# OpenRendererBenchmark/libYafaRay

Measured on AMD Instinct MI355X. Metric: Mrays/sec (primary+secondary) on the path-tracing hot path, higher is better.
Workload: dtype f32; 1 GPU; 1M-tri diffuse Cornell-box soup 512x512 64spp primary+1-bounce (BASELINE.json metric config); triangles=1000000, width=512, height=512, spp=64, bounces=1, lights=1, parallelism=pixel-tile shard x1, film_reduce=none, kd_nodes=2803313, kd_leaf_refs=3155999, kd_max_depth=27

## Files before the change

libyafaray_amd/csrc/yafgpu_device.hip:

```cpp
#include <hip/hip_runtime.h>

#include <algorithm>
#include <chrono>
#include <cmath>
#include <cstdio>
#include <cstdlib>
#include <cstring>
#include <string>
#include <vector>
#include <map>
#include <mutex>

#include "../../include/yafgpu.h"
#include "kdtree_build.h"
#include "yafgpu_math.h"
#include "yafgpu_shading.h"
#include "yafgpu_texture.h"

namespace yafgpu {

constexpr int kWave = 64;
constexpr int kBlock = 256;
constexpr int kWavesPerBlock = kBlock / kWave;
#ifndef YAFGPU_STACK
// ... 46 lines not shown
                                173, 179, 181, 191, 193, 197, 199, 211, 223, 227};

YG_DEV double scr_halton(const DevScene &sc, int dim, uint32_t n)
{
	double value = 0.0;
	const int *sigma = sc.faure + sc.faure_off[dim];
	const uint32_t base = (uint32_t)c_prims[dim];
	double f, factor, dn = (double)n;
	f = factor = sc.inv_prims[dim];
	while(n > 0)
	{
		value += (double)(sigma[n % base]) * factor;
		dn *= f;
		n = (uint32_t)dn;
		factor *= f;
	}
	return fmax(1.0e-36, fmin(1.0, value));
}

YG_DEV bool bound_cross(const DevScene &sc, V3 from, V3 dir, V3 inv_dir, float dist, float &enter, float &leave)
{
	const V3 a0 = mk(sc.blo[0], sc.blo[1], sc.blo[2]), a1 = mk(sc.bhi[0], sc.bhi[1], sc.bhi[2]);
	const V3 p = from - a0;
	float lmin = -1e38f, lmax = 1e38f, ltmin, ltmax;
	if(dir.x != 0.f)
	{
		const float inv = inv_dir.x;
		if(inv > 0.f) { lmin = -p.x * inv; lmax = ((a1.x - a0.x) - p.x) * inv; }
		else { lmin = ((a1.x - a0.x) - p.x) * inv; lmax = -p.x * inv; }
		if((lmax < 0.f) || (lmin > dist)) return false;
	}
	if(dir.y != 0.f)
	{
		const float inv = inv_dir.y;
		if(inv > 0.f) { ltmin = -p.y * inv; ltmax = ((a1.y - a0.y) - p.y) * inv; }
		else { ltmin = ((a1.y - a0.y) - p.y) * inv; ltmax = -p.y * inv; }
		lmin = smax(ltmin, lmin);
		lmax = smin(ltmax, lmax);
		if((lmax < 0.f) || (lmin > dist)) return false;
	}
	if(dir.z != 0.f)
	{
		const float inv = inv_dir.z;
		if(inv > 0.f) { ltmin = -p.z * inv; ltmax = ((a1.z - a0.z) - p.z) * inv; }
		else { ltmin = ((a1.z - a0.z) - p.z) * inv; ltmax = -p.z * inv; }
		lmin = smax(ltmin, lmin);
		lmax = smin(ltmax, lmax);
		if((lmax < 0.f) || (lmin > dist)) return false;
	}
	if((lmin <= lmax) && (lmax >= 0.f) && (lmin <= dist)) { enter = lmin; leave = lmax; return true; }
	return false;
}

YG_DEV bool tri_test(const float4 r0, const float4 r1, const float4 r2, V3 from, V3 dir, float &t, float &u, float &v)
{
	const V3 a = mk(r0.x, r0.y, r0.z), e1 = mk(r1.x, r1.y, r1.z), e2 = mk(r2.x, r2.y, r2.z);
	const float eps = r0.w;
	const V3 pvec = cross(dir, e2);
	const float det = dot(e1, pvec);
	if(det > -eps && det < eps) return false;
	const float inv_det = 1.f / det;
	const V3 tvec = from - a;
	u = dot(tvec, pvec) * inv_det;
	if(u < 0.f || u > 1.f) return false;
	const V3 qvec = cross(tvec, e1);
	v = dot(dir, qvec) * inv_det;
	if((v < 0.f) || ((u + v) > 1.f)) return false;
	t = dot(e2, qvec) * inv_det;
	if(t < eps) return false;
	return true;
}

YG_DEV bool tri_test_flat(const float4 r0, const float4 r1, const float4 r2, V3 from, V3 dir, float &t, float &u, float &v)
{
	const V3 a = mk(r0.x, r0.y, r0.z), e1 = mk(r1.x, r1.y, r1.z), e2 = mk(r2.x, r2.y, r2.z);
	const float eps = r0.w;
	const V3 pvec = cross(dir, e2);
	const float det = dot(e1, pvec);
	const bool det_ok = !(det > -eps && det < eps);
	const float inv_det = 1.f / det;
	const V3 tvec = from - a;
	u = dot(tvec, pvec) * inv_det;
	const bool u_ok = !(u < 0.f || u > 1.f);
	const V3 qvec = cross(tvec, e1);
	v = dot(dir, qvec) * inv_det;
	const bool v_ok = !((v < 0.f) || ((u + v) > 1.f));
	t = dot(e2, qvec) * inv_det;
	return det_ok && u_ok && v_ok && !(t < eps);
}

struct LaneStack
{
	uint2 *col;
	int sp, lo;
	YG_DEV void reset() { sp = 0; lo = 0; }
	YG_DEV bool empty() const { return sp == lo; }
	YG_DEV bool lost() const { return lo > 0; }
	YG_DEV void push(uint32_t node, float tmax)
	{
		col[(sp & (kStack - 1)) * kWave] = make_uint2(node, __float_as_uint(tmax));
		++sp;
		lo = max(lo, sp - kStack);
	}
	YG_DEV void pop(uint32_t &node, float &tmax)
	{
		--sp;
		const uint2 e = col[(sp & (kStack - 1)) * kWave];
		node = e.x; tmax = __uint_as_float(e.y);
	}
};

YG_DEV float restart_from(float tmin, float tmax)
{
	return (tmax > tmin) ? tmax : tmax + fmaxf(fabsf(tmax) * 1.2e-7f, 1e-30f);
}

YG_DEV void get_surface(const DevScene &sc, int ti, V3 hitp, float bu, float bv, SurfPt &sp)
{
	const float4 g = sc.tri_ng[ti];
	sp.ng = mk(g.x, g.y, g.z);
	if(sc.tri_vn != nullptr && __float_as_uint(g.w) != 0u)
	{
		const float u = 1.f - bu - bv, v = bu, w = bv;
		const float4 na = sc.tri_vn[3 * ti], nb = sc.tri_vn[3 * ti + 1], nc = sc.tri_vn[3 * ti + 2];
		sp.n = normalize(mk(na.x, na.y, na.z) * u + mk(nb.x, nb.y, nb.z) * v + mk(nc.x, nc.y, nc.z) * w);
	}
	else sp.n = sp.ng;
	sp.mat = (int)(__float_as_uint(sc.tri[3 * ti + 1].w) & 0x3FFFFFFFu);
	sp.p = hitp;
	create_cs(sp.n, sp.nu, sp.nv);
}

constexpr int kTsMaxDepth = 8;
YG_DEV bool kd_trace_ts(const DevScene &sc, LaneStack &stk, uint32_t *seen , V3 from, V3 dir, float ray_tmin, float dist,
                        int max_depth, Col &filt)
{
	filt = mkc(1.f, 1.f, 1.f);
	float a, b;
	if(sc.n_nodes == 0u) return false;
	const V3 inv_dir = mk(1.f / dir.x, 1.f / dir.y, 1.f / dir.z);
	if(!bound_cross(sc, from, dir, inv_dir, dist, a, b)) return false;
	const float t_exit = b;
	float tmin = smax(a, 0.f), tmax = t_exit;
	uint32_t node = 0u;
	int depth = 0, n_seen = 0;
	stk.reset();
	for(;;)
	{
		if(dist < tmin) break;
		uint2 nd = sc.nodes[node];
		while((nd.y & 3u) != 3u)
		{
			const int axis = (int)(nd.y & 3u);
			const float split = __uint_as_float(nd.x);
			const float o = comp(from, axis), d = comp(dir, axis);
			const float tplane = (split - o) * comp(inv_dir, axis);
			const bool below = (o < split) || (o == split && d <= 0.f);
			const uint32_t left = node + 1u, right = nd.y >> 2;
			const uint32_t near_c = below ? left : right, far_c = below ? right : left;
			if(!(tplane <= tmax) || tplane <= 0.f) node = near_c;
			else if(tplane < tmin) node = far_c;
			else { stk.push(far_c, tmax); node = near_c; tmax = tplane; }
			nd = sc.nodes[node];
		}
		const uint32_t np = nd.y >> 2, first = nd.x;
		for(uint32_t i = 0; i < np; ++i)
		{
			const uint32_t ti = sc.refs[first + i];
			const float4 r0 = sc.tri[3u * ti], r1 = sc.tri[3u * ti + 1u], r2 = sc.tri[3u * ti + 2u];
			float t, u, v;
			if(!tri_test(r0, r1, r2, from, dir, t, u, v)) continue;
			const uint32_t vis = __float_as_uint(r1.w) >> 30;
			if(!(t < dist && t >= ray_tmin && (vis == 0u || vis == 2u))) continue;
			const yafgpu_material &m = sc.mats[__float_as_uint(r1.w) & 0x3FFFFFFFu];
			if(!mat_is_transparent(m)) return true;
			bool known = false;
			for(int k = 0; k < n_seen; ++k) known = known || (seen[k * kWave] == ti);
			if(known) continue;
			if(depth >= max_depth) return true;
			if(n_seen <= kTsMaxDepth) seen[(n_seen++) * kWave] = ti;
			SurfPt sp;
			get_surface(sc, (int)ti, from + dir * t, u, v, sp);
			if(m.n_nodes > 0 && sc.tex.nodes != nullptr)
			{
				TexPoint tp; tex_point(sc.tex, (int)ti, u, v, sp.p, sp.n, sp.ng, tp);
				yafgpu_material tmp; mat_resolve(sc.tex, sc.cam, m, tp, tmp);
				filt = filt * mat_transparency(tmp, sp, dir);
			}
			else filt = filt * mat_transparency(m, sp, dir);
			++depth;
		}
		if(stk.empty())
		{
			if(!stk.lost() || tmax >= t_exit) break;
			tmin = restart_from(tmin, tmax); tmax = t_exit; node = 0u; stk.reset();
			continue;
		}
		tmin = tmax;
		stk.pop(node, tmax);
	}
	return false;
}

enum : int { kStPrimary = 0, kStFirst = 1, kStDepth = 2 };

YG_DEV int round2int(double v) { return (int)(v + (.5 - 1.4e-11)); }

YG_DEV uint32_t wave_sum(uint32_t v)
{
#pragma unroll
	for(int o = 32; o > 0; o >>= 1) v += __shfl_xor(v, o, kWave);
	return v;
}

}
#include "yafgpu_wavefront.h"
#ifndef YAFGPU_VARIANT_TU
namespace yafgpu {

__global__ __launch_bounds__(kBlock) void combine_kernel(const float *planes, float *film, int w, int h)
{
	const size_t n = (size_t)w * (size_t)h;
	const size_t stride = n * YAFGPU_FILM_CHANNELS;
	for(size_t i = (size_t)blockIdx.x * blockDim.x + threadIdx.x; i < n; i += (size_t)gridDim.x * blockDim.x)
	{
		const int x = (int)(i % (size_t)w), y = (int)(i / (size_t)w);
#pragma unroll
// ... 181 lines not shown
		}
		case 17:
		{
			if(n_in < 4) break;
			const uint32_t k = __float_as_uint(x[3]);
			if(k >= (uint32_t)sc.n_lights || sc.lights[k].type != YAFGPU_LIGHT_DIRECTIONAL || n_out < 8) break;
			Col c = mkc(0.f, 0.f, 0.f); V3 d = mk(0.f, 0.f, 0.f); float tmax = 0.f;
			const bool ok = directionallight_illuminate(sc.lights[k], mk(x[0], x[1], x[2]), c, d, tmax);
			o[0] = ok ? 1.f : 0.f;
			o[1] = ok ? d.x : 0.f; o[2] = ok ? d.y : 0.f; o[3] = ok ? d.z : 0.f; o[4] = ok ? tmax : 0.f; o[5] = ok ? c.r : 0.f; o[6] = ok ? c.g : 0.f; o[7] = ok ? c.b : 0.f;
			break;
		}
		case 18:
		{
			if(n_in < 3) break;
			const uint32_t k = __float_as_uint(x[2]);
			if(k >= (uint32_t)sc.n_lights || sc.lights[k].type != YAFGPU_LIGHT_SUN || n_out < 9) break;
			Col c = mkc(0.f, 0.f, 0.f); V3 d = mk(0.f, 0.f, 0.f); float tmax = 0.f, pdf = 0.f;
			const bool ok = sunlight_illum_sample(sc.lights[k], x[0], x[1], d, tmax, pdf, c);
			o[0] = ok ? 1.f : 0.f;
			o[1] = d.x; o[2] = d.y; o[3] = d.z; o[4] = tmax; o[5] = pdf; o[6] = c.r; o[7] = c.g; o[8] = c.b;
			break;
		}
		case 19:
		{
			if(n_in < 4) break;
			const uint32_t k = __float_as_uint(x[3]);
			if(k >= (uint32_t)sc.n_lights || sc.lights[k].type != YAFGPU_LIGHT_SUN || n_out < 6) break;
			Col c = mkc(0.f, 0.f, 0.f); float t = 0.f, ipdf = 0.f;
			const bool ok = sunlight_intersect(sc.lights[k], mk(x[0], x[1], x[2]), t, c, ipdf);
			o[0] = ok ? 1.f : 0.f; o[1] = t; o[2] = ipdf; o[3] = c.r; o[4] = c.g; o[5] = c.b;
			break;
		}
		case 20:
		{
			if(n_in < 6) break;
			const uint32_t k = __float_as_uint(x[5]);
			if(k >= (uint32_t)sc.n_lights || sc.lights[k].type != YAFGPU_LIGHT_SPHERE || n_out < 9) break;
			Col c = mkc(0.f, 0.f, 0.f); V3 d = mk(0.f, 0.f, 0.f); float tmax = 0.f, pdf = 0.f;
			const bool ok = spherelight_illum_sample(sc.lights[k], mk(x[0], x[1], x[2]), x[3], x[4], d, tmax, pdf, c);
			o[0] = ok ? 1.f : 0.f;
			o[1] = ok ? d.x : 0.f; o[2] = ok ? d.y : 0.f; o[3] = ok ? d.z : 0.f; o[4] = ok ? tmax : 0.f; o[5] = ok ? pdf : 0.f;
			o[6] = ok ? c.r : 0.f; o[7] = ok ? c.g : 0.f; o[8] = ok ? c.b : 0.f;
			break;
		}
		case 21:
		{
			if(n_in < 7) break;
			const uint32_t k = __float_as_uint(x[6]);
			if(k >= (uint32_t)sc.n_lights || sc.lights[k].type != YAFGPU_LIGHT_SPHERE || n_out < 3) break;
			float d_1 = 0.f, d_2 = 0.f;
			const bool ok = sphere_intersect(mk(x[0], x[1], x[2]), mk(x[3], x[4], x[5]), vec3(sc.lights[k].position), sc.lights[k].square_radius, d_1, d_2);
			o[0] = ok ? 1.f : 0.f; o[1] = d_1; o[2] = ok ? d_2 : 0.f;
			break;
		}
		default: break;
	}
}

}

using namespace yafgpu;

static float host_fsin(float x);
static thread_local std::string g_err;
static int fail(int code, const std::string &msg) { g_err = msg; return code; }
#define HIP_OK(expr) do { hipError_t e_ = (expr); if(e_ != hipSuccess) return fail(-100, std::string(#expr) + ": " + hipGetErrorString(e_)); } while(0)

template<typename T> struct DevMem
{
	T *p = nullptr; size_t cap = 0;
	DevMem() = default;
	DevMem(const DevMem &) = delete; DevMem &operator=(const DevMem &) = delete;
	~DevMem() { if(p) (void)hipFree(p); }
	hipError_t alloc(size_t count) { return hipMalloc((void **)&p, std::max<size_t>(count, 1) * sizeof(T)); }
	hipError_t reserve(size_t count, hipStream_t stream)
	{
		if(p && count <= cap) return hipSuccess;
		hipError_t e = hipStreamSynchronize(stream);
		if(e != hipSuccess) return e;
		if(p) (void)hipFree(p);
		p = nullptr; cap = 0;
		if((e = alloc(count)) != hipSuccess) { p = nullptr; return e; }
		cap = count;
		return hipSuccess;
	}
	operator T *() const { return p; }
};
struct Stream
{
	hipStream_t s = nullptr;
	Stream() = default;
	Stream(const Stream &) = delete; Stream &operator=(const Stream &) = delete;
	~Stream() { if(s) (void)hipStreamDestroy(s); }
	hipError_t create() { return s ? hipSuccess : hipStreamCreateWithFlags(&s, hipStreamNonBlocking); }
	operator hipStream_t() const { return s; }
};
struct Event
{
	hipEvent_t e = nullptr;
	Event() = default;
	Event(const Event &) = delete; Event &operator=(const Event &) = delete;
	~Event() { if(e) (void)hipEventDestroy(e); }
	hipError_t create(unsigned flags = hipEventDisableTiming) { return e ? hipSuccess : hipEventCreateWithFlags(&e, flags); }
	operator hipEvent_t() const { return e; }
};
// ... 137 lines not shown
	}
	auto *s = new yafgpu_scene();
	{
		std::vector<char> used((size_t)d->n_materials, 0);
		for(int i = 0; i < d->n_tris; ++i) used[(size_t)d->tri_mat[i]] = 1;
		for(int i = 0; i < d->n_materials; ++i)
		{
			if(!used[(size_t)i]) continue;
			const yafgpu_material &m = d->materials[i];
			s->mat_mask |= 1u << (uint32_t)m.type;
			if(m.bsdf_flags & kVolumetric) s->has_volumetric = true;
			if(m.bsdf_flags & (kSpecular | kFilter)) s->has_specular = true;
			if(m.anisotropic) s->has_aniso = true;
			s->max_add_depth = std::max(s->max_add_depth, std::min(std::max(m.additional_depth, 0), 15));
			if(m.bsdf_flags & kGlossy) s->has_glossy = true;
			if(m.type == YAFGPU_MAT_ROUGH_GLASS) s->has_glossy_two = true;
			if((m.type == YAFGPU_MAT_SHINYDIFFUSE && m.is_transparent) || ((m.type == YAFGPU_MAT_GLASS || m.type == YAFGPU_MAT_ROUGH_GLASS) && m.fake_shadow)) s->has_transparent = true;
		}
	}
	const auto t0 = std::chrono::steady_clock::now();
	{
		bool on_device = d->build_on_device > 0 || (d->build_on_device == 0 && d->n_tris >= 65536);
		if(const char *e = std::getenv("YAFGPU_BUILD")) on_device = std::strcmp(e, "device") == 0;
		if(on_device)
		{
			std::string err;
			const int brc = build_kdtree_device_retry(d->verts, d->n_tris, kDepthCap, s->tree, &err);
			if(brc == -2 || brc == -3) build_kdtree(d->verts, d->n_tris, kDepthCap, d->build_threads, s->tree);
			else if(brc) { delete s; return fail(-20, err); }
		}
		else build_kdtree(d->verts, d->n_tris, kDepthCap, d->build_threads, s->tree);
	}
	s->info.build_seconds = s->tree.build_seconds;
	s->info.n_nodes = (uint32_t)s->tree.nodes.size();
	s->info.n_leaf_refs = (uint32_t)s->tree.refs.size();
	s->info.max_depth = (uint32_t)s->tree.max_depth;
	s->info.n_tris = (uint32_t)d->n_tris;
	const auto t1 = std::chrono::steady_clock::now();

	const size_t nt = (size_t)d->n_tris;
	std::vector<float4> rec(3 * nt), ng(nt), vn;
	bool any_smooth = false;
	for(size_t i = 0; i < nt; ++i)
	{
		const float *v = d->verts + 9 * i;
		const float e1[3] = {v[3] - v[0], v[4] - v[1], v[5] - v[2]}, e2[3] = {v[6] - v[0], v[7] - v[1], v[8] - v[2]};
		const float l1 = std::sqrt(e1[0] * e1[0] + e1[1] * e1[1] + e1[2] * e1[2]);
		const float l2 = std::sqrt(e2[0] * e2[0] + e2[1] * e2[1] + e2[2] * e2[2]);
		const float eps = (float)((double)0.1f * 0.00005 * (double)std::max(l1, l2));
		const uint32_t mat = (uint32_t)d->tri_mat[i];
		const uint32_t vis = (uint32_t)d->materials[mat].visibility & 3u;
		float mw; const uint32_t packed = mat | (vis << 30); std::memcpy(&mw, &packed, 4);
		rec[3 * i] = make_float4(v[0], v[1], v[2], eps);
		rec[3 * i + 1] = make_float4(e1[0], e1[1], e1[2], mw);
		rec[3 * i + 2] = make_float4(e2[0], e2[1], e2[2], 0.f);
		float n[3] = {e1[1] * e2[2] - e1[2] * e2[1], e1[2] * e2[0] - e1[0] * e2[2], e1[0] * e2[1] - e1[1] * e2[0]};
		float len = n[0] * n[0] + n[1] * n[1] + n[2] * n[2];
		if(len != 0.f) { len = 1.0f / std::sqrt(len); n[0] *= len; n[1] *= len; n[2] *= len; }
		bool smooth = false;
		if(d->vnormals)
		{
			const float *q = d->vnormals + 9 * i;
			for(int k = 0; k < 9; ++k) if(q[k] != 0.f) smooth = true;
		}
		float sw; const uint32_t sbits = smooth ? 1u : 0u; std::memcpy(&sw, &sbits, 4);
		ng[i] = make_float4(n[0], n[1], n[2], sw);
		any_smooth |= smooth;
	}
	if(any_smooth)
	{
		vn.resize(3 * nt);
		for(size_t i = 0; i < nt; ++i)
		{
			const float *q = d->vnormals + 9 * i;
			for(int c = 0; c < 3; ++c)
			{
				float x = q[3 * c], y = q[3 * c + 1], z = q[3 * c + 2];
				if(x == 0.f && y == 0.f && z == 0.f) { x = ng[i].x; y = ng[i].y; z = ng[i].z; }
				vn[3 * i + (size_t)c] = make_float4(x, y, z, 0.f);
			}
		}
	}
	std::vector<int> faure; std::vector<int> foff(50); std::vector<double> invp(50);
	for(int dim = 0; dim < 50; ++dim)
	{
		foff[(size_t)dim] = (int)faure.size();
		std::vector<int> p;
		if(dim < 3) p = {0, 1, 2};
		else faure_perm(kPrimsHost[dim], p);
		faure.insert(faure.end(), p.begin(), p.end());
		char buf[32];
		std::snprintf(buf, sizeof buf, "%.9f", 1.0 / (double)kPrimsHost[dim]);
		invp[(size_t)dim] = std::strtod(buf, nullptr);
	}
	int rc = 0;
	DevScene &dv = s->dev;
	if((rc = upload(s, (const uint2 *)s->tree.nodes.data(), s->tree.nodes.size(), &dv.nodes))) { yafgpu_scene_destroy(s); return rc; }
	{
		const char *e = std::getenv("YAFGPU_TREELET_INLINE");
		TreeletLayout tl;
		if(build_treelets(s->tree.nodes, !(e && std::atoi(e) == 0), tl)) { yafgpu_scene_destroy(s); return fail(-2, "kd-tree too large for the treelet layout"); }
		dv.tl_root = tl.root;
		if((rc = upload(s, (const uint4 *)tl.words.data(), tl.words.size() / 4, &dv.treelets))) { yafgpu_scene_destroy(s); return rc; }
		if((rc = upload(s, (const uint2 *)tl.leaves.data(), tl.leaves.size() / 2, &dv.tl_leaves))) { yafgpu_scene_destroy(s); return rc; }
	}
	if((rc = upload(s, s->tree.refs.data(), s->tree.refs.size(), &dv.refs))) { yafgpu_scene_destroy(s); return rc; }
	if((rc = upload(s, rec.data(), rec.size(), &dv.tri))) { yafgpu_scene_destroy(s); return rc; }
	if((rc = upload(s, ng.data(), ng.size(), &dv.tri_ng))) { yafgpu_scene_destroy(s); return rc; }
// ... 1274 lines not shown
```

libyafaray_amd/csrc/yafgpu_wavefront.h:

```cpp
#pragma once

namespace yafgpu {

constexpr int kWfRecs = 32;

struct WfArgs
{
	RenderArgs ra;
	float4 *state; uint32_t cap;
	float4 *results;
	uint32_t n_paths, pixel_begin, n_pixels;
	const uint32_t *pix_prefix;
	int frames;
	int frame_recs, has_glossy;
	int pix_listed;
	uint32_t *pix_xy;
	const uint32_t *q_closest_in, *q_shadow_in, *q_resume_in;
	uint32_t *q_closest_out, *q_shadow_out, *q_resume_out;
	uint32_t *verdict;
	float4 *shadow_filt;
	int replay, replay_lights;
	int ev_m;
	float4 *hit_cache; int hit_k;
	uint32_t *ev_flags;
// ... 91 lines not shown
		}
		return true;
	}
	r_tmin = ra.rp.min_raydist_auto ? ra.ray_min_dist * smax(1.f, length(sp.p)) : ra.ray_min_dist;
	float W = 0.f;
	BsdfSample bs; bs.s_1 = s_1; bs.s_2 = s_2; bs.pdf = 0.f; bs.flags = kMisFlags; bs.sampled = kNone;
	const Col surf_col = mat_sample(mat, dat, sp, wo, r_dir, bs, W);
	float light_ipdf;
	Col l_col = mkc(0.f, 0.f, 0.f);
	if(YG_LIGHT_IS(light, YAFGPU_LIGHT_SUN)) { if(!(bs.pdf > 1e-6f && sunlight_intersect(light, r_dir, r_tmax, l_col, light_ipdf))) return false; }
	else if(YG_LIGHT_IS(light, YAFGPU_LIGHT_SPHERE)) return false;
	else if(!(bs.pdf > 1e-6f && arealight_intersect(light, sp.p, r_dir, r_tmax, light_ipdf))) return false;
	if(light_ipdf > 1e-6f)
	{
		const float l_pdf = 1.f / light_ipdf;
		const float l_2 = l_pdf * l_pdf, m_2 = bs.pdf * bs.pdf;
		const float w = m_2 / (l_2 + m_2);
		contrib = ((surf_col * (YG_LIGHT_IS(light, YAFGPU_LIGHT_SUN) ? l_col : col3(light.color))) * w) * W;
	}
	return true;
}

YG_DEV float4 &wf_rec(const WfArgs &a, int k, uint32_t slot)
{
	return *(float4 *)((char *)(a.state + (size_t)k * a.cap) + (slot << 4));
}
#define REC(k) wf_rec(a, (k), slot)
YG_DEV uint32_t wf_event(const WfArgs &a, uint32_t slot, uint32_t z19, int path_i)
{
	const uint32_t call = a.ev_m > 1 ? min(z19 >> 24, (uint32_t)a.ev_m - 1u) : 0u;
	return (slot * (uint32_t)a.ev_m + call) * (uint32_t)max(a.ra.rp.path_samples, 1) + (uint32_t)path_i;
}

YG_DEV const yafgpu_material &wf_mat_hit(const DevScene &sc, const SurfPt &sp, int tri, float bu, float bv, yafgpu_material &tmp)
{
	const yafgpu_material &m = sc.mats[sp.mat];
#if YAFGPU_FEAT_TEXTURE
	if(m.n_nodes > 0 && sc.tex.nodes != nullptr)
	{
		TexPoint tp; tex_point(sc.tex, tri, bu, bv, sp.p, sp.n, sp.ng, tp);
		mat_resolve(sc.tex, sc.cam, m, tp, tmp);
		return tmp;
	}
#endif
	return m;
}
YG_DEV bool wf_bump_hit(const DevScene &sc, SurfPt &sp, int tri, float bu, float bv)
{
#if YAFGPU_FEAT_TEXTURE
	const yafgpu_material &m = sc.mats[sp.mat];
	if(m.n_bump <= 0 || !sc.tex.has_bump) return false;
	TexPoint tp; tex_point(sc.tex, tri, bu, bv, sp.p, sp.n, sp.ng, tp);
	const float4 r1 = sc.tri[3 * tri + 1], r2 = sc.tri[3 * tri + 2];
	tex_point_derivatives(sc.tex, tri, mk(r1.x, r1.y, r1.z), mk(r2.x, r2.y, r2.z), sp.n, sp.nu, sp.nv, tp);
	NodeResult stack[kMaxNodes];
	nodes_eval_derivative(sc.tex, sc.tex.nodes + m.bump_first, min(m.n_bump, kMaxNodes), sc.cam, tp, stack);
	apply_bump(sp.n, sp.nu, sp.nv, stack[m.sh_bump].col.r, stack[m.sh_bump].col.g);
	return true;
#else
	(void)sc; (void)sp; (void)tri; (void)bu; (void)bv;
	return false;
#endif
}
YG_DEV void wf_frame_set(SurfPt &sp, const float4 nu)
{
	if(nu.w != 0.f) { sp.nu = v3(nu); sp.nv = normalize(cross(sp.n, sp.nu)); }
}
YG_DEV void wf_frame_parked(const WfArgs &a, uint32_t slot, int vertex, SurfPt &sp)
{
#if YAFGPU_FEAT_TEXTURE
	if(a.ra.sc.tex.has_bump) wf_frame_set(sp, REC(24 + vertex));
#else
	(void)a; (void)slot; (void)vertex; (void)sp;
#endif
}
YG_DEV const yafgpu_material &wf_mat_parked(const WfArgs &a, uint32_t slot, int vertex, const SurfPt &sp, yafgpu_material &tmp)
{
	const yafgpu_material &m = a.ra.sc.mats[sp.mat];
#if YAFGPU_FEAT_TEXTURE
	if(m.n_nodes > 0 && a.ra.sc.tex.nodes != nullptr)
	{
		const float4 r = REC(22 + vertex);
		return wf_mat_hit(a.ra.sc, sp, (int)ubits(r.x), r.y, r.z, tmp);
	}
#endif
	return m;
}

struct Ctl { Col col; int pc, stage, dl_on_sp0, depth, path_i, level, incl, add, mask2; };
YG_DEV uint32_t pack_ctl(const Ctl &c) { return (uint32_t)c.pc | ((uint32_t)c.stage << 2) | ((uint32_t)c.dl_on_sp0 << 4) | ((uint32_t)c.level << 5) | ((uint32_t)c.depth << 8) | ((uint32_t)c.add << 12) | ((uint32_t)c.incl << 16) | (((uint32_t)c.path_i & 0x1fffu) << 17) | ((uint32_t)c.mask2 << 30); }
YG_DEV Ctl load_ctl(const WfArgs &a, uint32_t slot)
{
	const float4 r = REC(13);
	const uint32_t w = ubits(r.w);
	Ctl c; c.col = c3(r);
	c.pc = (int)(w & 3u); c.stage = (int)((w >> 2) & 3u); c.dl_on_sp0 = (int)((w >> 4) & 1u); c.level = (int)((w >> 5) & 7u);
	c.depth = (int)((w >> 8) & 0xfu); c.add = (int)((w >> 12) & 0xfu); c.incl = (int)((w >> 16) & 1u); c.path_i = (int)((w >> 17) & 0x1fffu); c.mask2 = (int)(w >> 30);
	return c;
}
YG_DEV uint32_t pack_dlc(int li, int l_end, int mask, int is) { return (uint32_t)li | ((uint32_t)l_end << 8) | ((uint32_t)mask << 16) | ((uint32_t)is << 20); }

enum { W_AFTER_CLOSEST, W_AFTER_SHADOW, W_DL_NEXT, W_DL_EVAL, W_DL_DONE, W_RECURSE, W_RETURN, W_EXTEND, W_START_PATH, W_FINISH, W_PARK_CLOSEST, W_PARK_SHADOW,
       W_GLOSSY_NEXT, W_RECURSE_SPEC, W_PARK_BOTH, W_NEXT_VERTEX };

#ifndef YAFGPU_HOT_ACC
#define YAFGPU_HOT_ACC 1
#endif
// ... 1073 lines not shown
		float4 *b = a.state + slot; const size_t c = a.cap;
		b[0 * c] = f4(from, tmin);
		b[1 * c] = f4(dir, tmax);
		b[13 * c] = make_float4(0.f, 0.f, 0.f, fbits((uint32_t)kPcAfterClosest | ((uint32_t)kStPrimary << 2)));
	}
	if(blockIdx.x == 0 && threadIdx.x == 0) { a.cnt_in[0] = a.n_paths; a.cnt_in[1] = 0u; a.cnt_in[2] = 0u; a.cnt_in[3] = 0u; a.cnt_in[4] = 0u; }
}

#ifndef YAFGPU_VOTE_NUM
#define YAFGPU_VOTE_NUM 1
#endif
#ifndef YAFGPU_VOTE_DEN
#define YAFGPU_VOTE_DEN 1
#endif
#ifndef YAFGPU_NODE_BURST
#define YAFGPU_NODE_BURST 2
#endif
#ifndef YAFGPU_TRACE_BATCH
#define YAFGPU_TRACE_BATCH 512
#endif
constexpr int kTraceBatch = YAFGPU_TRACE_BATCH;
#ifndef YAFGPU_REFILL
#define YAFGPU_REFILL 24
#endif
#ifndef YAFGPU_TRACE_POSTPONE
#define YAFGPU_TRACE_POSTPONE 1
#endif
#ifndef YAFGPU_TRACE_BELOW_MASKS
#define YAFGPU_TRACE_BELOW_MASKS 1
#endif
#ifndef YAFGPU_TRACE_WAVES
#define YAFGPU_TRACE_WAVES 7
#endif
template<bool kAny, bool kStats>
__global__ __launch_bounds__(kBlock, YAFGPU_TRACE_WAVES) void wf_trace(const WfArgs a)
{
	__shared__ uint2 s_stack[kWavesPerBlock][kStack][kWave];
	__shared__ float2 s_axis[kWavesPerBlock][3][kWave];
	const int lane = (int)(threadIdx.x & (kWave - 1)), wave = (int)(threadIdx.x >> 6);
	const DevScene &sc = a.ra.sc;
	const uint32_t root = sc.tl_root;
	LaneStack stk;
	stk.col = &s_stack[wave][0][lane];
	float2 *const axis_col = &s_axis[wave][0][lane];
	LaneCounters cn = {0u, 0u, 0u, 0u, 0u, 0u, 0u};
	const uint32_t n = kAny ? a.cnt_in[1] : a.cnt_in[0];
	uint32_t *cursor = kAny ? &a.cnt_in[3] : &a.cnt_in[2];
	const uint32_t *q = kAny ? a.q_shadow_in : a.q_closest_in;
	const size_t c = a.cap;
	bool exhausted = (n == 0u);
	uint32_t slot = 0u, link = 0u, which = 0u, pair = 0u, qi = 0u;
	uint32_t w_next = 0u, w_end = 0u;
	const uint32_t batch = min((uint32_t)kTraceBatch, max((uint32_t)kWave, (n / (gridDim.x * (uint32_t)kWavesPerBlock * 2u)) & ~63u));
	V3 from = mk(0.f, 0.f, 0.f), dir = from;
	uint32_t dneg = 0u;
	float ray_tmin = 0.f, dist = 0.f, t_exit = 0.f, tmin = 0.f, tmax = 0.f, z = 0.f, bu = 0.f, bv = 0.f;
	int tri = -1; bool hit = false;
	auto answer_any = [&](bool occluded) {
		const uint32_t bit = 4u * slot + 2u * pair + which;
		if(occluded) atomicOr(&a.verdict[bit >> 5], 1u << (bit & 31u));
	};
	enum : uint32_t { kWalk = 0u, kBlocked = 1u, kWalkEnd = 2u, kNoRay = 3u };
	constexpr int kVoteNum = YAFGPU_VOTE_NUM, kVoteDen = YAFGPU_VOTE_DEN, kNodeBurst = YAFGPU_NODE_BURST;
	uint32_t ws = kNoRay;
	uint32_t p_cur = 0u, p_end = 0u, ti = 0u;
	float p_tmax = 0.f;
	bool done = false;
	uint32_t spec = 0u;
	uint32_t spec_leaves = 0u;
	uint32_t rounds_node = 0u, rounds_tri = 0u;
	for(;;)
	{
		const unsigned long long idle = __ballot(ws == kNoRay);
		const int n_idle = __popcll(idle);
		if(!exhausted && (n_idle >= YAFGPU_REFILL || n_idle == kWave))
		{
			if(w_next >= w_end)
			{
				const int leader = __ffsll((long long)idle) - 1;
				uint32_t base = 0u;
				if(lane == leader) base = atomicAdd(cursor, batch);
				base = (uint32_t)__shfl((int)base, leader, kWave);
				w_next = base; w_end = min(base + batch, n);
				if(base >= n) { exhausted = true; w_next = w_end = 0u; }
			}
			const uint32_t avail = w_end - w_next;
			const uint32_t rank = (uint32_t)__popcll(idle & ((1ull << lane) - 1ull));
			const uint32_t first_i = w_next;
			w_next += min(avail, (uint32_t)n_idle);
			if(ws == kNoRay && rank < avail)
			{
				const uint32_t i = first_i + rank;
				slot = q ? q[i] : i;
				qi = i;
				which = slot >> 31;
				pair = kAny ? (slot >> 30) & 1u : 0u;
				slot &= kAny ? 0x3fffffffu : 0x7fffffffu;
				float4 r0 = a.state[slot], r1 = a.state[c + slot];
				if(!kAny && which)
				{
					const float4 r26 = a.state[26 * c + slot];
					r1 = make_float4(r26.x, r26.y, r26.z, -1.f);
					r0.w = r26.w;
				}
				if(kAny && pair)
				{
					const float4 ra_ = a.state[(which ? 30 : 28) * c + slot];
					const float rb_ = a.state[(which ? 31 : 29) * c + slot].w;
					r1 = make_float4(ra_.x, ra_.y, ra_.z, which ? rb_ : ra_.w);
					r0.w = which ? ra_.w : rb_;
				}
				else if(kAny && which)
				{
					const float4 r20 = a.state[20 * c + slot];
					r1 = make_float4(r20.x, r20.y, r20.z, a.state[21 * c + slot].w);
					r0.w = r20.w;
				}
				from = v3(r0); dir = v3(r1);
				if(kAny)
				{
					from = from + dir * r0.w;
					dist = (r1.w < 0.f) ? INFINITY : r1.w - 2.f * r0.w;
					ray_tmin = a.ra.rp.transp_shad ? r0.w : 0.f;
					++cn.shadow;
				}
				else
				{
					dist = (r1.w < 0.f) ? INFINITY : r1.w;
					ray_tmin = r0.w;
					++cn.closest;
				}
				float ea, eb;
				tri = -1; hit = false; z = dist; bu = 0.f; bv = 0.f; done = false; p_cur = p_end = 0u;
				const V3 inv_dir = mk(1.f / dir.x, 1.f / dir.y, 1.f / dir.z);
				if(sc.n_nodes != 0u && bound_cross(sc, from, dir, inv_dir, dist, ea, eb) && !(dist < smax(ea, 0.f)))
				{
					axis_col[0] = make_float2(from.x, inv_dir.x);
					axis_col[kWave] = make_float2(from.y, inv_dir.y);
					axis_col[2 * kWave] = make_float2(from.z, inv_dir.z);
					dneg = (dir.x <= 0.f ? 1u : 0u) | (dir.y <= 0.f ? 2u : 0u) | (dir.z <= 0.f ? 4u : 0u);
					t_exit = eb; tmin = smax(ea, 0.f); tmax = t_exit; link = root; ws = kWalk;
					stk.reset();
				}
				else
				{
					if(!kAny) a.state[2 * c + qi] = make_float4(fbits(0xffffffffu), dist, 0.f, 0.f);
				}
			}
		}
		const unsigned long long m_act = __ballot(ws != kNoRay);
		if(m_act == 0ull) { if(exhausted) break; else continue; }
		const bool has_pend = p_cur < p_end;
		const unsigned long long m_tri = __ballot(has_pend);
		const int n_tri = __popcll(m_tri), n_node = __popcll(__ballot(ws == kWalk));
		auto leaf_end = [&]() {
			const uint2 top = stk.col[((stk.sp - 1) & (kStack - 1)) * kWave];
			const bool hit_here = !kAny && hit && z <= tmax;
			const bool emp = stk.empty();
			const bool restart = emp && stk.lost() && !(tmax >= t_exit);
			if(kStats && restart && !hit_here) ++cn.restarts;
			tmin = restart ? restart_from(tmin, tmax) : tmax;
			link = emp ? root : top.x;
			tmax = emp ? t_exit : __uint_as_float(top.y);
			stk.sp = emp ? 0 : stk.sp - 1;
			stk.lo = emp ? 0 : stk.lo;
			const bool fin = hit_here || (emp && !restart) || z < tmin;
			ws = fin ? kWalkEnd : kWalk;
		};
		auto tri_step = [&](const float4 r0, const float4 r1, const float4 r2, const uint32_t ref_v) {
			float t, u, v;
			if(kStats) ++cn.tests;
			const bool ok = tri_test_flat(r0, r1, r2, from, dir, t, u, v);
			const uint32_t vis = __float_as_uint(r1.w) >> 30;
			if(kAny)
			{
				const bool found = ok && t < dist && t >= ray_tmin && (vis == 0u || vis == 2u);
				hit = hit || found; done = done || found;
			}
			else
			{
				const bool better = ok && t < z && t >= ray_tmin && (vis == 0u || vis == 1u);
				z = better ? t : z; tri = better ? (int)ti : tri; bu = better ? u : bu; bv = better ? v : bv; hit = hit || better;
			}
			++p_cur; ti = ref_v;
			if(p_cur >= p_end)
			{
				if(YAFGPU_TRACE_POSTPONE)
				{
					const bool ends = !kAny && hit && z <= p_tmax;
					done = done || ends;
					if(kStats) { if(done) { cn.interior -= spec; cn.leaves -= spec_leaves; } spec = 0u; spec_leaves = 0u; }
					if(!kAny && ws != kWalkEnd && z < tmin) ws = kWalkEnd;
					ws = (ws == kBlocked) ? kWalk : ws;
				}
				else if(!done) leaf_end();
			}
		};
		auto node_step = [&](const uint4 t0, const uint4 t1) {
			const uint32_t sl = link & 3u;
			const uint32_t axis = (t0.w >> (2u * sl)) & 3u;
			const float split = __uint_as_float(sl == 0u ? t0.x : (sl == 1u ? t0.y : t0.z));
			const float2 oi = axis_col[axis * kWave];
			const float o = oi.x;
			const float tplane = (split - o) * oi.y;
			const bool dn = ((dneg >> axis) & 1u) != 0u;
#if YAFGPU_TRACE_BELOW_MASKS
			const bool below = __builtin_amdgcn_inverse_ballot_w64(__ballot(o < split) | (__ballot(o == split) & __ballot(dn)));
#else
			const bool below = dn ? (o <= split) : (o < split);
#endif
			const bool l_in = sl == 0u && ((t0.w >> 2) & 3u) != 3u, r_in = sl == 0u && ((t0.w >> 4) & 3u) != 3u;
			const uint32_t left = l_in ? (link | 1u) : (sl == 2u ? t1.z : t1.x);
			const uint32_t right = r_in ? (link | 2u) : (sl == 0u ? t1.z : (sl == 1u ? t1.y : t1.w));
			const uint32_t near_c = below ? left : right, far_c = below ? right : left;
			if(kStats) { ++cn.interior; if(p_cur < p_end) ++spec; }
			const bool near_only = !(tplane <= tmax) || tplane <= 0.f;
			const bool far_only = !near_only && tplane < tmin;
			const bool both = !near_only && !far_only;
			stk.col[(stk.sp & (kStack - 1)) * kWave] = make_uint2(far_c, __float_as_uint(tmax));
			stk.sp += both ? 1 : 0;
			stk.lo = max(stk.lo, stk.sp - (kStack - 1));
			link = far_only ? far_c : near_c;
			tmax = both ? tplane : tmax;
		};
		auto leaf_step = [&]() {
			uint32_t first = link & ((1u << kLinkFirstBits) - 1u), np = (link >> kLinkFirstBits) & kLinkCountMax;
			if(link & kLinkEscape) { const uint2 e = sc.tl_leaves[link & kLinkIndex]; first = e.x; np = e.y; }
			if(np == 0u) { if(kStats) { ++cn.leaves; if(p_cur < p_end) ++spec_leaves; } leaf_end(); }
			else if(!YAFGPU_TRACE_POSTPONE)
			{
				if(kStats) ++cn.leaves;
				p_cur = first; p_end = first + np; p_tmax = tmax; ti = sc.refs[first]; ws = kBlocked;
			}
			else if(p_cur < p_end) ws = kBlocked;
			else
			{
				if(kStats) ++cn.leaves;
				p_cur = first; p_end = first + np; p_tmax = tmax;
				ti = sc.refs[first];
				leaf_end();
			}
		};
		if(n_tri * kVoteNum >= n_node * kVoteDen && n_tri > 0)
		{
			if(kStats) ++rounds_tri;
			if(has_pend)
			{
				uint32_t ref_v = 0u;
				if(p_cur + 1u < p_end) ref_v = sc.refs[p_cur + 1u];
				const float4 r0 = sc.tri[3u * ti], r1 = sc.tri[3u * ti + 1u], r2 = sc.tri[3u * ti + 2u];
				tri_step(r0, r1, r2, ref_v);
			}
		}
		else
		{
#pragma unroll 1
			for(int s = 0; s < kNodeBurst; ++s)
			{
				if(kStats && __ballot(ws == kWalk) != 0ull) ++rounds_node;
				if(ws == kWalk && (link & kLinkLeaf)) leaf_step();
				const bool fetch = ws == kWalk && !(link & kLinkLeaf);
				const uint32_t at = link >> 2;
				uint4 t0 = make_uint4(0u, 0u, 0u, 0u), t1 = t0;
				if(fetch) { t0 = sc.treelets[2u * at]; t1 = sc.treelets[2u * at + 1u]; }
				if(fetch) node_step(t0, t1);
				if(ws == kWalk && (link & kLinkLeaf)) leaf_step();
				if(fetch && ws == kWalk && (link >> 2) == at) node_step(t0, t1);
			}
		}
		if(done || (ws == kWalkEnd && p_cur >= p_end))
		{
			if(kAny) answer_any(hit);
			else a.state[2 * c + qi] = make_float4(fbits((uint32_t)(hit ? tri : -1)), z, bu, bv);
			ws = kNoRay; done = false; p_cur = p_end = 0u;
		}
	}
	if(a.ra.counters != nullptr)
	{
		const uint32_t v0 = wave_sum(cn.closest), v1 = wave_sum(cn.shadow), v2 = wave_sum(cn.interior), v3_ = wave_sum(cn.leaves),
		               v4 = wave_sum(cn.tests), v6 = wave_sum(cn.restarts);
		if(lane == 0 && (v0 | v1))
		{
			if(v0) atomicAdd((unsigned long long *)&a.ra.counters->rays_closest, (unsigned long long)v0);
			if(v1) atomicAdd((unsigned long long *)&a.ra.counters->rays_shadow, (unsigned long long)v1);
			if(kStats)
			{
				atomicAdd((unsigned long long *)&a.ra.counters->interior_steps, (unsigned long long)v2);
				atomicAdd((unsigned long long *)&a.ra.counters->leaves, (unsigned long long)v3_);
				atomicAdd((unsigned long long *)&a.ra.counters->tri_tests, (unsigned long long)v4);
				atomicAdd((unsigned long long *)&a.ra.counters->restarts, (unsigned long long)v6);
				atomicAdd((unsigned long long *)&a.ra.counters->wave_rounds, (unsigned long long)rounds_node | ((unsigned long long)rounds_tri << 32));
			}
		}
	}
}


__global__ __launch_bounds__(kBlock) void wf_trace_ts(const WfArgs a)
{
	__shared__ uint2 s_stack[kWavesPerBlock][kStack][kWave];
	__shared__ uint32_t s_seen[kWavesPerBlock][kTsMaxDepth + 1][kWave];
	const int lane = (int)(threadIdx.x & (kWave - 1)), wave = (int)(threadIdx.x >> 6);
	const DevScene &sc = a.ra.sc;
	LaneStack stk;
// ... 404 lines not shown
```

Measured before the change: 2561 Mrays/s.

## Interleave triangle edge components and use packed float2 math in ray-triangle test

Reorders the triangle record so edge1/edge2 components are interleaved per axis, with the material/visibility word moved into the third float4. The wavefront tri test now computes the pvec/qvec crosses and dots two lanes at a time using float2 vectors, so the compiler can emit packed FP32 instructions. Loading now uses 8-byte reads instead of a full third float4. Ray direction is kept inside the packed vectors rather than as a separate V3. A debug test case compares the scalar and packed results. The risks are extra swizzle overhead and slightly different rounding.

```diff
diff --git a/libyafaray_amd/csrc/yafgpu_device.hip b/libyafaray_amd/csrc/yafgpu_device.hip
--- a/libyafaray_amd/csrc/yafgpu_device.hip
+++ b/libyafaray_amd/csrc/yafgpu_device.hip
@@ -122,9 +122,16 @@
 	return false;
 }
 
+YG_DEV void tri_edges(const float4 r1, const float4 r2, V3 &e1, V3 &e2)
+{
+	e1 = mk(r1.x, r1.z, r2.x); e2 = mk(r1.y, r1.w, r2.y);
+}
+YG_DEV uint32_t tri_mat_vis(const float4 r2) { return __float_as_uint(r2.z); }
+
 YG_DEV bool tri_test(const float4 r0, const float4 r1, const float4 r2, V3 from, V3 dir, float &t, float &u, float &v)
 {
-	const V3 a = mk(r0.x, r0.y, r0.z), e1 = mk(r1.x, r1.y, r1.z), e2 = mk(r2.x, r2.y, r2.z);
+	const V3 a = mk(r0.x, r0.y, r0.z);
+	V3 e1, e2; tri_edges(r1, r2, e1, e2);
 	const float eps = r0.w;
 	const V3 pvec = cross(dir, e2);
 	const float det = dot(e1, pvec);
@@ -141,21 +148,24 @@
 	return true;
 }
 
-YG_DEV bool tri_test_flat(const float4 r0, const float4 r1, const float4 r2, V3 from, V3 dir, float &t, float &u, float &v)
-{
-	const V3 a = mk(r0.x, r0.y, r0.z), e1 = mk(r1.x, r1.y, r1.z), e2 = mk(r2.x, r2.y, r2.z);
-	const float eps = r0.w;
-	const V3 pvec = cross(dir, e2);
-	const float det = dot(e1, pvec);
+typedef float f32x2 __attribute__((ext_vector_type(2)));
+YG_DEV bool tri_test_pk(const float4 a_eps, const f32x2 ex, const f32x2 ey, const f32x2 ez, V3 from, f32x2 tdx, f32x2 tdy, f32x2 tdz,
+                        float &t, float &u, float &v)
+{
+	const float eps = a_eps.w;
+	tdx.x = from.x - a_eps.x; tdy.x = from.y - a_eps.y; tdz.x = from.z - a_eps.z;
+	const f32x2 qpx = tdy * ez - tdz * ey, qpy = tdz * ex - tdx * ez, qpz = tdx * ey - tdy * ex;
+	const f32x2 pqx = qpx.yx, pqy = qpy.yx, pqz = qpz.yx;
+	const f32x2 det_t = (ex * pqx + ey * pqy) + ez * pqz;
+	const f32x2 uv = (tdx * pqx + tdy * pqy) + tdz * pqz;
+	const float det = det_t.x;
 	const bool det_ok = !(det > -eps && det < eps);
 	const float inv_det = 1.f / det;
-	const V3 tvec = from - a;
-	u = dot(tvec, pvec) * inv_det;
+	const f32x2 uv_s = uv * inv_det;
+	u = uv_s.x; v = uv_s.y;
 	const bool u_ok = !(u < 0.f || u > 1.f);
-	const V3 qvec = cross(tvec, e1);
-	v = dot(dir, qvec) * inv_det;
 	const bool v_ok = !((v < 0.f) || ((u + v) > 1.f));
-	t = dot(e2, qvec) * inv_det;
+	t = det_t.y * inv_det;
 	return det_ok && u_ok && v_ok && !(t < eps);
 }
 
@@ -196,7 +206,7 @@
 		sp.n = normalize(mk(na.x, na.y, na.z) * u + mk(nb.x, nb.y, nb.z) * v + mk(nc.x, nc.y, nc.z) * w);
 	}
 	else sp.n = sp.ng;
-	sp.mat = (int)(__float_as_uint(sc.tri[3 * ti + 1].w) & 0x3FFFFFFFu);
+	sp.mat = (int)(tri_mat_vis(sc.tri[3 * ti + 2]) & 0x3FFFFFFFu);
 	sp.p = hitp;
 	create_cs(sp.n, sp.nu, sp.nv);
 }
@@ -240,9 +250,9 @@
 			const float4 r0 = sc.tri[3u * ti], r1 = sc.tri[3u * ti + 1u], r2 = sc.tri[3u * ti + 2u];
 			float t, u, v;
 			if(!tri_test(r0, r1, r2, from, dir, t, u, v)) continue;
-			const uint32_t vis = __float_as_uint(r1.w) >> 30;
+			const uint32_t vis = tri_mat_vis(r2) >> 30;
 			if(!(t < dist && t >= ray_tmin && (vis == 0u || vis == 2u))) continue;
-			const yafgpu_material &m = sc.mats[__float_as_uint(r1.w) & 0x3FFFFFFFu];
+			const yafgpu_material &m = sc.mats[tri_mat_vis(r2) & 0x3FFFFFFFu];
 			if(!mat_is_transparent(m)) return true;
 			bool known = false;
 			for(int k = 0; k < n_seen; ++k) known = known || (seen[k * kWave] == ti);
@@ -530,6 +540,21 @@
 			float d_1 = 0.f, d_2 = 0.f;
 			const bool ok = sphere_intersect(mk(x[0], x[1], x[2]), mk(x[3], x[4], x[5]), vec3(sc.lights[k].position), sc.lights[k].square_radius, d_1, d_2);
 			o[0] = ok ? 1.f : 0.f; o[1] = d_1; o[2] = ok ? d_2 : 0.f;
+			break;
+		}
+		case 22:
+		{
+			if(n_in < 16 || n_out < 8) break;
+			const V3 from = mk(x[0], x[1], x[2]), dir = mk(x[3], x[4], x[5]);
+			const float4 r0 = make_float4(x[6], x[7], x[8], x[15]), r1 = make_float4(x[9], x[12], x[10], x[13]), r2 = make_float4(x[11], x[14], 0.f, 0.f);
+			float t = 0.f, u = 0.f, v = 0.f;
+			const bool ok = tri_test(r0, r1, r2, from, dir, t, u, v);
+			o[0] = ok ? 1.f : 0.f; o[1] = t; o[2] = u; o[3] = v;
+			f32x2 ex, ey, ez, tdx, tdy, tdz;
+			ex.x = r1.x; ex.y = r1.y; ey.x = r1.z; ey.y = r1.w; ez.x = r2.x; ez.y = r2.y;
+			tdx.x = 0.f; tdx.y = dir.x; tdy.x = 0.f; tdy.y = dir.y; tdz.x = 0.f; tdz.y = dir.z;
+			const bool ok_pk = tri_test_pk(r0, ex, ey, ez, from, tdx, tdy, tdz, t, u, v);
+			o[4] = ok_pk ? 1.f : 0.f; o[5] = t; o[6] = u; o[7] = v;
 			break;
 		}
 		default: break;
@@ -773,8 +798,8 @@
 		const uint32_t vis = (uint32_t)d->materials[mat].visibility & 3u;
 		float mw; const uint32_t packed = mat | (vis << 30); std::memcpy(&mw, &packed, 4);
 		rec[3 * i] = make_float4(v[0], v[1], v[2], eps);
-		rec[3 * i + 1] = make_float4(e1[0], e1[1], e1[2], mw);
-		rec[3 * i + 2] = make_float4(e2[0], e2[1], e2[2], 0.f);
+		rec[3 * i + 1] = make_float4(e1[0], e2[0], e1[1], e2[1]);
+		rec[3 * i + 2] = make_float4(e1[2], e2[2], mw, 0.f);
 		float n[3] = {e1[1] * e2[2] - e1[2] * e2[1], e1[2] * e2[0] - e1[0] * e2[2], e1[0] * e2[1] - e1[1] * e2[0]};
 		float len = n[0] * n[0] + n[1] * n[1] + n[2] * n[2];
 		if(len != 0.f) { len = 1.0f / std::sqrt(len); n[0] *= len; n[1] *= len; n[2] *= len; }
diff --git a/libyafaray_amd/csrc/yafgpu_wavefront.h b/libyafaray_amd/csrc/yafgpu_wavefront.h
--- a/libyafaray_amd/csrc/yafgpu_wavefront.h
+++ b/libyafaray_amd/csrc/yafgpu_wavefront.h
@@ -167,7 +167,8 @@
 	if(m.n_bump <= 0 || !sc.tex.has_bump) return false;
 	TexPoint tp; tex_point(sc.tex, tri, bu, bv, sp.p, sp.n, sp.ng, tp);
 	const float4 r1 = sc.tri[3 * tri + 1], r2 = sc.tri[3 * tri + 2];
-	tex_point_derivatives(sc.tex, tri, mk(r1.x, r1.y, r1.z), mk(r2.x, r2.y, r2.z), sp.n, sp.nu, sp.nv, tp);
+	V3 e1, e2; tri_edges(r1, r2, e1, e2);
+	tex_point_derivatives(sc.tex, tri, e1, e2, sp.n, sp.nu, sp.nv, tp);
 	NodeResult stack[kMaxNodes];
 	nodes_eval_derivative(sc.tex, sc.tex.nodes + m.bump_first, min(m.n_bump, kMaxNodes), sc.cam, tp, stack);
 	apply_bump(sp.n, sp.nu, sp.nv, stack[m.sh_bump].col.r, stack[m.sh_bump].col.g);
@@ -1347,7 +1348,8 @@
 	uint32_t slot = 0u, link = 0u, which = 0u, pair = 0u, qi = 0u;
 	uint32_t w_next = 0u, w_end = 0u;
 	const uint32_t batch = min((uint32_t)kTraceBatch, max((uint32_t)kWave, (n / (gridDim.x * (uint32_t)kWavesPerBlock * 2u)) & ~63u));
-	V3 from = mk(0.f, 0.f, 0.f), dir = from;
+	V3 from = mk(0.f, 0.f, 0.f);
+	f32x2 tdx = {0.f, 0.f}, tdy = tdx, tdz = tdx;
 	uint32_t dneg = 0u;
 	float ray_tmin = 0.f, dist = 0.f, t_exit = 0.f, tmin = 0.f, tmax = 0.f, z = 0.f, bu = 0.f, bv = 0.f;
 	int tri = -1; bool hit = false;
@@ -1411,7 +1413,9 @@
 					r1 = make_float4(r20.x, r20.y, r20.z, a.state[21 * c + slot].w);
 					r0.w = r20.w;
 				}
-				from = v3(r0); dir = v3(r1);
+				from = v3(r0);
+				const V3 dir = v3(r1);
+				tdx.y = dir.x; tdy.y = dir.y; tdz.y = dir.z;
 				if(kAny)
 				{
 					from = from + dir * r0.w;
@@ -1462,11 +1466,11 @@
 			const bool fin = hit_here || (emp && !restart) || z < tmin;
 			ws = fin ? kWalkEnd : kWalk;
 		};
-		auto tri_step = [&](const float4 r0, const float4 r1, const float4 r2, const uint32_t ref_v) {
+		auto tri_step = [&](const float4 r0, const f32x2 ex, const f32x2 ey, const f32x2 ez, const uint32_t mat_vis, const uint32_t ref_v) {
 			float t, u, v;
 			if(kStats) ++cn.tests;
-			const bool ok = tri_test_flat(r0, r1, r2, from, dir, t, u, v);
-			const uint32_t vis = __float_as_uint(r1.w) >> 30;
+			const bool ok = tri_test_pk(r0, ex, ey, ez, from, tdx, tdy, tdz, t, u, v);
+			const uint32_t vis = mat_vis >> 30;
 			if(kAny)
 			{
 				const bool found = ok && t < dist && t >= ray_tmin && (vis == 0u || vis == 2u);
@@ -1543,8 +1547,11 @@
 			{
 				uint32_t ref_v = 0u;
 				if(p_cur + 1u < p_end) ref_v = sc.refs[p_cur + 1u];
-				const float4 r0 = sc.tri[3u * ti], r1 = sc.tri[3u * ti + 1u], r2 = sc.tri[3u * ti + 2u];
-				tri_step(r0, r1, r2, ref_v);
+				const float4 *rec = sc.tri + 3u * (size_t)ti;
+				const float4 r0 = rec[0];
+				const f32x2 ex = *(const f32x2 *)((const float *)rec + 4), ey = *(const f32x2 *)((const float *)rec + 6), ez = *(const f32x2 *)((const float *)rec + 8);
+				const uint32_t mat_vis = *((const uint32_t *)rec + 10);
+				tri_step(r0, ex, ey, ez, mat_vis, ref_v);
 			}
 		}
 		else
```

Measured after the change: 2624 Mrays/s (median of 6 runs). 1.02x the previous value.
